# Fe0437/CudaVolumeRenderer

Measured on AMD Instinct MI355X. Metric: Msamples/sec + achieved HBM GB/s, manix.vdb 1024x1024 @ 1/2/4/8 MI355X, higher is better.
Workload: dtype f32

## Files before the change

### cudavolumerenderer_amd/csrc/cvr_wpool.hip

```cpp
#include <hip/hip_runtime.h>

#include "cvr_env.h"
#include "cvr_kernels.h"
#include "cvr_walk.h"

#ifndef CVR_WPOOL_UNROLL
#define CVR_WPOOL_UNROLL 4
#endif
#ifndef CVR_WPOOL_EMASK
#define CVR_WPOOL_EMASK 1
#endif
#ifndef CVR_WPOOL_SPARSE_WPG
#define CVR_WPOOL_SPARSE_WPG 4
#endif
#ifndef CVR_WPOOL_DENSE_WPG
#define CVR_WPOOL_DENSE_WPG 1
#endif
#ifndef CVR_WPOOL_LOOK
#define CVR_WPOOL_LOOK 2
#endif
#ifndef CVR_WPOOL_SPARSE_DEFER
#define CVR_WPOOL_SPARSE_DEFER 1
#endif
#ifndef CVR_WPOOL_TAILSTAMP
#define CVR_WPOOL_TAILSTAMP 0
#endif
constexpr int kLook = CVR_WPOOL_LOOK;
static_assert(CVR_WPOOL_UNROLL >= kLook && CVR_WPOOL_UNROLL % kLook == 0,
              "CVR_WPOOL_UNROLL must be a positive multiple of kLook");
constexpr int kPrioTrack = 1, kPrioEvent = 0;

namespace cvr {

namespace {

__device__ __forceinline__ float opaque_s(float x) {
  asm volatile("" : "+s"(x));
  return x;
}

constexpr int kLdsGranule = 1280;
template <int kWaves, int kExtra = 0, int kWpg = 1>
struct PoolSize {
  static_assert((4 * kWaves) % kWpg == 0, "a CU's waves split into whole workgroups");
  static constexpr int kBudget = 163840 / (4 * kWaves / kWpg) / kLdsGranule * kLdsGranule;
  static constexpr int kParams = (int)((sizeof(LaunchParams) + 15) / 16 * 16);
  static constexpr int value = ((kBudget - kParams - kExtra) / kWpg - 24 - 4 * STAT_COUNT) / 64;
  static_assert(4 * STAT_COUNT + 8 + 12 + 4 <= 4 * STAT_COUNT + 24, "pool header exceeds its LDS reserve");
};
constexpr int kWpgSparse = CVR_WPOOL_SPARSE_WPG, kWpgDense = CVR_WPOOL_DENSE_WPG;
constexpr int wpg_of(int kMedMk, int kWaves) {
  return (kMedMk & 3) != 1  ? ((4 * kWaves) % kWpgDense == 0 ? kWpgDense : 1)
                                            : ((4 * kWaves) % kWpgSparse == 0 ? kWpgSparse : 4);
}

template <int kSlots>
struct WavePool {
  float4 a[kSlots], b[kSlots];
  uint4 c[kSlots];
  uint2 e[kSlots];
  uint32_t meta[kSlots];
  uint8_t ready[kSlots];
  uint8_t lb[kSlots];
  uint8_t lc[kSlots];
  uint8_t ln[kSlots];
  uint32_t cnt[STAT_COUNT];
  unsigned long long dead;
  uint32_t cur[3];
  uint32_t pend;
};
constexpr uint32_t kCurExhausted = 1u << 16;

__device__ __forceinline__ uint32_t lane_rank(unsigned long long mask) {
  return __builtin_amdgcn_mbcnt_hi((uint32_t)(mask >> 32), __builtin_amdgcn_mbcnt_lo((uint32_t)mask, 0u));
}

__device__ __forceinline__ uint32_t normal_code(V3 n) {
  return n.x > 0.f ? 1u : n.x < 0.f ? 2u : n.y > 0.f ? 3u : n.y < 0.f ? 4u : n.z > 0.f ? 5u : n.z < 0.f ? 6u : 0u;
}
__device__ __forceinline__ V3 normal_of(uint32_t c) {
  const float s = (c & 1u) ? 1.0f : -1.0f;
  return c == 0u ? mk3(0, 0, 0) : c <= 2u ? mk3(s, 0, 0) : c <= 4u ? mk3(0, s, 0) : mk3(0, 0, s);
}

template <class Pool>
__device__ __forceinline__ void store_full(Pool& S, float4* __restrict__ gT, uint32_t s,
                                           const PathState& ps, const Isect& is, uint32_t nseg,
                                           uint32_t wword) {
  S.a[s] = make_float4(ps.o.x, ps.o.y, ps.o.z, 0.0f);
  S.b[s] = make_float4(ps.d.x, ps.d.y, ps.d.z, is.dist);
  S.c[s] = make_uint4(ps.rng.v0, ps.rng.v1, ps.rng.v2, ps.rng.v3);
  S.e[s] = make_uint2(ps.rng.v4, ps.rng.d);
  S.meta[s] = normal_code(is.normal) | (is.inside ? 8u : 0u) | (nseg << 4);
  gstore4(gT + s, make_float4(ps.T.x, ps.T.y, ps.T.z, __uint_as_float(wword)));
}
template <class Pool>
__device__ __forceinline__ void load_full(const Pool& S, const float4* __restrict__ gT, uint32_t s,
                                          PathState& ps, Isect& is, uint32_t& nseg, float& t) {
  const float4 f = gload4(gT + s);
  const float4 a = S.a[s], b = S.b[s];
  const uint4 c = S.c[s];
  const uint2 e = S.e[s];
  const uint32_t meta = S.meta[s];
  ps.o = mk3(a.x, a.y, a.z);
  t = a.w;
  ps.d = mk3(b.x, b.y, b.z);
  is.dist = b.w;
  ps.T = mk3(f.x, f.y, f.z);
  ps.rng = Rng{c.x, c.y, c.z, c.w, e.x, e.y};
  ps.image_id = __float_as_uint(f.w);
  is.normal = normal_of(meta & 7u);
  is.inside = (meta & 8u) != 0u;
  nseg = meta >> 4;
}
template <class Pool>
__device__ __forceinline__ void store_track(Pool& S, uint32_t s, float t, const Rng& rng) {
  S.a[s].w = t;
  S.c[s] = make_uint4(rng.v0, rng.v1, rng.v2, rng.v3);
  S.e[s] = make_uint2(rng.v4, rng.d);
}
template <class Pool>
__device__ __forceinline__ void load_track(const Pool& S, uint32_t s, V3& o, V3& d, Rng& rng, float& t,
                                           float& max_t) {
  const float4 a = S.a[s], b = S.b[s];
  const uint4 c = S.c[s];
  const uint2 e = S.e[s];
  o = mk3(a.x, a.y, a.z);
  t = a.w;
  d = mk3(b.x, b.y, b.z);
  max_t = b.w;
  rng = Rng{c.x, c.y, c.z, c.w, e.x, e.y};
}

typedef __attribute__((address_space(3))) const LaunchParams LdsParams;
__device__ __forceinline__ const LaunchParams& fresh(const LaunchParams& L) {
  LdsParams* p = (LdsParams*)&L;
  asm volatile("" : "+v"(p));
  return *(const LaunchParams*)p;
}

enum : uint32_t { K_BOUNDARY = 0, K_COLLIDE = 1, K_NEW = 2, K_NONE = 3 };

template <bool kCombine, class Pool>
__device__ __forceinline__ void splat_wave(Pool& S, const LaunchParams& L, const PathState& ps, bool esc,
                                           uint32_t s, uint32_t lane) {
#if defined(CVR_DIAG_NO_SPLAT)
  (void)S; (void)L; (void)ps; (void)esc; (void)s; (void)lane;
  return;
#endif
  unsigned long long rest = __ballot(esc);
  if (rest == 0ull) return;
  if (!kCombine || !(fresh(L).wflags & kSplatCombine)) {
    if (esc) splat(L, ps);
    return;
  }
  uint32_t leader = lane;
  bool multi = false;
  while (rest != 0ull) {
    const uint32_t l0 = (uint32_t)__builtin_ctzll(rest);
    const uint32_t id0 = __builtin_amdgcn_readlane(ps.image_id, l0);
    const unsigned long long g = __ballot(esc && ps.image_id == id0);
    if (esc && ps.image_id == id0) leader = l0;
    multi |= (g & (g - 1ull)) != 0ull;
    rest &= ~g;
  }
  if (!multi) {
    if (esc) splat(L, ps);
    return;
  }
  const uint32_t sl = (uint32_t)__shfl((int)s, (int)leader);
  float* acc = reinterpret_cast<float*>(&S.a[sl]);
  const bool lead = esc && leader == lane;
  if (lead) {
    acc[0] = ps.T.x;
    acc[1] = ps.T.y;
    acc[2] = ps.T.z;
  }
  asm volatile("s_waitcnt lgkmcnt(0)" ::: "memory");
  if (esc && !lead) {
    __hip_atomic_fetch_add(acc + 0, ps.T.x, __ATOMIC_RELAXED, __HIP_MEMORY_SCOPE_WORKGROUP);
    __hip_atomic_fetch_add(acc + 1, ps.T.y, __ATOMIC_RELAXED, __HIP_MEMORY_SCOPE_WORKGROUP);
    __hip_atomic_fetch_add(acc + 2, ps.T.z, __ATOMIC_RELAXED, __HIP_MEMORY_SCOPE_WORKGROUP);
  }
  asm volatile("s_waitcnt lgkmcnt(0)" ::: "memory");
  if (lead) {
    PathState q{};
    q.image_id = ps.image_id;
    q.T = mk3(acc[0], acc[1], acc[2]);
    splat(L, q);
  }
}

template <int kSlots, int kWpg>
__device__ __forceinline__ uint32_t* rec_pids(const LaunchParams& L, uint32_t gw) {
  return reinterpret_cast<uint32_t*>(L.rec) - (size_t)gridDim.x * kWpg * kSlots + (size_t)gw * kSlots;
}
template <int kSlots, int kWpg>
__device__ __forceinline__ void record_end(const LaunchParams& L, uint32_t gw, uint32_t s, const PathState& ps,
                                           uint32_t flags, uint32_t nseg) {
  const uint32_t pid = rec_pids<kSlots, kWpg>(L, gw)[s];
  PathRecord r = {};
  r.image_id = ps.image_id;
  r.flags = flags;
  r.T[0] = ps.T.x;
  r.T[1] = ps.T.y;
  r.T[2] = ps.T.z;
  r.n_segments = nseg;
  static_cast<PathRecord*>(L.rec)[pid - L.path_first] = r;
}



constexpr unsigned kWaitVm0 = 0x0F70;
constexpr uint32_t kPendAgg = 0x80000000u;

template <class Pool>
__device__ __forceinline__ uint32_t count_ended(const Pool& S, const LaunchParams& L, uint32_t pend,
                                                uint32_t lane) {
#if defined(CVR_DIAG_NO_COUNT)
  (void)S; (void)L; (void)pend; (void)lane;
  return 0u;
#endif
  const uint32_t base = pend & 0xFFu, n = pend >> 8;
#if !defined(CVR_DIAG_NO_COUNT_WAIT)
  __builtin_amdgcn_s_waitcnt(kWaitVm0);
#endif
  uint32_t blk = 0;
  if (lane < n) blk = tile_block_of(fresh(L), S.meta[S.ln[base + lane]]);
  const uint32_t b0 = __builtin_amdgcn_readfirstlane(blk);
  const unsigned long long same = __ballot(lane < n && blk == b0);
  const bool rest = lane < n && blk != b0;
  const unsigned long long rm = __ballot(rest);
  if (rm != 0ull) {
    const uint32_t first = (uint32_t)__builtin_ctzll(rm);
    const uint32_t b1 = __builtin_amdgcn_readlane(blk, first);
    const unsigned long long s1 = __ballot(rest && blk == b1);
    if (lane == first || (rest && blk != b1))
      __hip_atomic_fetch_add(gmem(fresh(L).frame_done + kDoneStride * blk), lane == first ? (unsigned int)__popcll(s1) : 1u,
                             __ATOMIC_RELAXED, __HIP_MEMORY_SCOPE_AGENT);
  }
  return kPendAgg | b0 << 7 | (uint32_t)__popcll(same);
}
__device__ __forceinline__ void add_counted(const LaunchParams& L, uint32_t agg) {
#if defined(CVR_DIAG_NO_COUNT)
  (void)L; (void)agg;
  return;
#endif
  __hip_atomic_fetch_add(gmem(fresh(L).frame_done + kDoneStride * ((agg & ~kPendAgg) >> 7)), agg & 0x7Fu,
                         __ATOMIC_RELAXED, __HIP_MEMORY_SCOPE_AGENT);
}

__device__ __forceinline__ void store_blocks(const LaunchParams& L, const FrameFlush& F, const uint32_t (&b)[8], uint32_t nb,
                                             uint32_t lane) {
  float v[8][3];
  size_t pix[8];
#pragma unroll
  for (uint32_t k = 0; k < 8u; ++k) {
    if (k < nb) {
      const uint32_t by = fastdiv(b[k], L.div_blocks_x), bx = b[k] - by * L.blocks_x;
      const uint32_t px = bx * 8u + (lane & 7u), py = by * 8u + (lane >> 3);
      pix[k] = (size_t)py * L.tile_w + px;
      gptr_t<float> src = gmem(reinterpret_cast<float*>(L.out + pix[k]));
#pragma unroll
      for (int c = 0; c < 3; ++c) v[k][c] = __hip_atomic_fetch_add(src + c, 0.0f, __ATOMIC_RELAXED, __HIP_MEMORY_SCOPE_AGENT);
    }
  }
#pragma unroll
  for (uint32_t k = 0; k < 8u; ++k) {
    if (k < nb) {
      const float x = v[k][0], y = v[k][1], z = v[k][2];
      const float w = (x != 0.0f || y != 0.0f || z != 0.0f) ? 1.0f : 0.0f;
      float4* dst = F.host + pix[k];
      __builtin_nontemporal_store(x / F.scale, &dst->x);
      __builtin_nontemporal_store(y / F.scale, &dst->y);
      __builtin_nontemporal_store(z / F.scale, &dst->z);
      __builtin_nontemporal_store(w / F.scale, &dst->w);
    }
  }
}

constexpr unsigned long long kFlushPatience = 100000000ull;
constexpr unsigned int kFlushed = 0x80000000u;
__device__ void frame_flusher(const LaunchParams& L, uint32_t f, uint32_t lane) {
  const FrameFlush F = *frame_header(L.frame_done);
  if (F.give_up) {
    if (lane == 0) __hip_atomic_store(F.status + kFrameFlushers, 1u, __ATOMIC_RELAXED, __HIP_MEMORY_SCOPE_SYSTEM);
    return;
  }
  const uint32_t quota = 64u * L.samples, qi = lane & 7u, off = lane >> 3, q = f + kFrameFlushers * qi;
  uint32_t cur = 0, end = 0, stored = 0;
  if (q < L.n_queues) {
    cur = queue_blocks_begin(L, q);
    end = queue_blocks_begin(L, q + 1u);
  }
  unsigned long long last = __builtin_amdgcn_s_memrealtime();
  for (;;) {
    if (__ballot(cur < end) == 0ull) break;
    const bool mine = cur + off < end;
    uint32_t tb = 0, v = 0;
    if (mine) {
      tb = launch_block_tile(L, cur + off);
      v = __hip_atomic_fetch_add(gmem(L.frame_done + kDoneStride * tb), 0u, __ATOMIC_RELAXED, __HIP_MEMORY_SCOPE_AGENT);
    }
    const bool ready = mine && v < kFlushed && v >= quota;
    unsigned long long rm = __ballot(ready);
    const unsigned long long settled = __ballot(mine && v >= quota);
    const unsigned long long now = __builtin_amdgcn_s_memrealtime();
    const bool any_ready = rm != 0ull;
    while (rm != 0ull) {
      uint32_t bsel[8], nb = 0;
#pragma unroll
      for (uint32_t k = 0; k < 8u; ++k) {
        if (rm != 0ull) {
          bsel[k] = __builtin_amdgcn_readlane(tb, (uint32_t)__builtin_ctzll(rm));
          rm &= rm - 1ull;
          ++nb;
        }
      }
      store_blocks(L, F, bsel, nb, lane);
      stored += nb;
    }
    if (ready) __hip_atomic_fetch_or(gmem(L.frame_done + kDoneStride * tb), kFlushed, __ATOMIC_RELAXED, __HIP_MEMORY_SCOPE_AGENT);
    uint32_t lead = 0;
#pragma unroll
    for (uint32_t o = 0; o < 8u; ++o)
      if (lead == o && ((settled >> (qi + 8u * o)) & 1ull)) ++lead;
    cur += lead;
    if (any_ready) {
      last = now;
    } else if (__ballot(lead != 0u) == 0ull) {
      if (now - last > kFlushPatience) {
        if (lane == 0) __hip_atomic_store(F.status + kFrameFlushers, 1u, __ATOMIC_RELAXED, __HIP_MEMORY_SCOPE_SYSTEM);
        break;
      }
      __builtin_amdgcn_s_sleep(32);
    }
  }
  if (lane == 0) __hip_atomic_store(F.status + f, stored, __ATOMIC_RELAXED, __HIP_MEMORY_SCOPE_SYSTEM);
}


}

#if CVR_WPOOL_TAILSTAMP
constexpr uint32_t kTailWaves = 16384;
__device__ unsigned long long g_tail[8 * kTailWaves];
#endif
static_assert(sizeof(LaunchParams) == 256 && sizeof(MediumParams) == 256,
              "the moments buffer is addressed from LaunchParams::out: the parameter structs keep their size");
__device__ __forceinline__ void splat_moments(const LaunchParams& L, const PathState& ps) {
  gptr_t<float> px = gmem(reinterpret_cast<float*>(L.out + L.tile_px + ps.image_id));
  const float xx = ps.T.x * ps.T.x, yy = ps.T.y * ps.T.y, zz = ps.T.z * ps.T.z;
  if (xx != 0.0f) __hip_atomic_fetch_add(px + 0, xx, __ATOMIC_RELAXED, __HIP_MEMORY_SCOPE_AGENT);
  if (yy != 0.0f) __hip_atomic_fetch_add(px + 1, yy, __ATOMIC_RELAXED, __HIP_MEMORY_SCOPE_AGENT);
  if (zz != 0.0f) __hip_atomic_fetch_add(px + 2, zz, __ATOMIC_RELAXED, __HIP_MEMORY_SCOPE_AGENT);
  __hip_atomic_fetch_add(px + 3, 1.0f, __ATOMIC_RELAXED, __HIP_MEMORY_SCOPE_AGENT);
}
__device__ __forceinline__ void env_shade(const LaunchParams& L, PathState& ps) {
  typedef __attribute__((address_space(4))) const uint32_t* CWords;
  const uint64_t a = reinterpret_cast<uint64_t>(fresh(L).rec);
  const uint32_t lo = (uint32_t)__builtin_amdgcn_readfirstlane((uint32_t)a);
  const uint32_t hi = (uint32_t)__builtin_amdgcn_readfirstlane((uint32_t)(a >> 32));
  const uint64_t ua = (uint64_t)lo | (uint64_t)hi << 32;
  CWords hw = reinterpret_cast<CWords>(ua);
  EnvParams E;
  E.texels = reinterpret_cast<const float4*>((uint64_t)hw[0] | (uint64_t)hw[1] << 32);
  E.w = hw[2];
  E.h = hw[3];
#pragma unroll
  for (int i = 0; i < 9; ++i) E.R[i] = __uint_as_float(hw[4 + i]);
  float rgb[3];
  env_lookup(E, ps.d.x, ps.d.y, ps.d.z, rgb);
  ps.T = mk3(ps.T.x * rgb[0], ps.T.y * rgb[1], ps.T.z * rgb[2]);
}
template <bool kScatterEps, int kWaves, int kMedMk, bool kRecord, bool kFlush>
__global__ __launch_bounds__(64 * wpg_of(kMedMk, kWaves), kWaves) void k_wpool(MediumParams mk, LaunchParams Lk) {
  constexpr bool kMK = (kMedMk & kMedMK) != 0;
  constexpr bool kCountWords = (kMedMk & kMedCount) != 0;
  constexpr bool kMoments = (kMedMk & kMedMoments) != 0;
  constexpr bool kEnv = (kMedMk & kMedEnv) != 0;
  constexpr int kMed = kMedMk & 3;
  static_assert(!kEnv || (kWaves == kWpoolWaves && !kMK && !kRecord && !kFlush && !kCountWords),
                "environment: the default budget, no naiveMK walk, records, in-launch output or word counts");
  static_assert(!kMoments || (!kMK && !kRecord && !kFlush && !kCountWords && !(kMedMk & kMedHalf)),
                "moments: no naiveMK walk, records, in-launch output, word counts or pinned half format");
  static_assert(!kMK || (kScatterEps && !kRecord && !kFlush), "naiveMK: scatter -eps, no records / in-launch output");
  constexpr bool kSparse = kMed == kMedSparse;
  constexpr bool kLookDefer = kSparse && CVR_WPOOL_SPARSE_DEFER;
  constexpr int kEm = kSparse && CVR_WPOOL_EMASK ? kEmaskWords : 0;
  constexpr int kWpg = wpg_of(kMedMk, kWaves);
  constexpr int kSlots = PoolSize<kWaves, 4 * kEm, kWpg>::value;
  if constexpr (kFlush && kWpg == 1) {
    if (Lk.frame_done != nullptr && blockIdx.x < kFrameFlushers) {
      frame_flusher(Lk, blockIdx.x, threadIdx.x);
      return;
    }
  }
  const uint32_t wv = kWpg > 1 ? __builtin_amdgcn_readfirstlane(threadIdx.x >> 6) : 0u;
  const uint32_t gw = blockIdx.x * (uint32_t)kWpg + wv;
  MediumParams m = mk;
  if constexpr (!kSparse) {
    m.leaves = nullptr;
    m.leaf_density = nullptr;
    m.leaf_albedo = nullptr;
    m.sbounds = nullptr;
    if constexpr (kMed == kMedDenseFull || kMed == kMedDenseFullUniform) {
      __builtin_assume(m.cells != nullptr);
      __builtin_assume(m.bounds != nullptr);
      m.albedo_uniform = kMed == kMedDenseFullUniform ? 1u : 0u;
      m.format = (kMedMk & kMedHalf) ? 1u : 0u;
    }
  } else {
    m.density = nullptr;
    m.albedo = nullptr;
    m.bounds = nullptr;
    __builtin_assume(m.leaves != nullptr);
    __builtin_assume(m.sbounds != nullptr);
    m.albedo_uniform = 0u;
    m.format = (kMedMk & kMedHalf) ? 1u : 0u;
  }
  static_assert(!(kMedMk & kMedHalf) || kMed != kMedDense, "the generic dense instance reads the format at run time");
#if CVR_WPOOL_TAILSTAMP
  const unsigned long long ts_start = __builtin_amdgcn_s_memrealtime();
  unsigned long long ts_ex = 0, ts_ev = 0, ts_a = 0;
  uint32_t ts_live = 0, ts_batches = 0, ts_trk = 0, ts_steps0 = 0, ts_seg0 = 0;
#endif
  static_assert(kWpg * sizeof(WavePool<kSlots>) + 4 * kEm + sizeof(LaunchParams) <=
                    (size_t)PoolSize<kWaves, 0, kWpg>::kBudget,
                "wave pools exceed the LDS budget of kWaves waves per SIMD");
  static_assert(kSlots <= 256, "the pool's rings and stacks hold slot indices as uint8_t");
  __shared__ WavePool<kSlots> Sw[kWpg];
  WavePool<kSlots>& S = Sw[wv];
  __shared__ uint32_t EM[kEm ? kEm : 1];
  __shared__ LaunchParams L;
  const uint32_t lane = kWpg > 1 ? threadIdx.x & 63u : threadIdx.x;
  if (threadIdx.x == 0) L = Lk;
  if constexpr (kEm != 0) {
    for (uint32_t i = threadIdx.x; i < (uint32_t)kEm; i += 64u * kWpg) EM[i] = m.emask ? m.emask[i] : ~0u;
  }
  __syncthreads();
  if constexpr (kFlush && kWpg > 1) {
    if (Lk.frame_done != nullptr && gw < kFrameFlushers) {
      frame_flusher(Lk, gw, lane);
      return;
    }
  }
  uint32_t c_steps = 0, c_fetch = 0;
  uint32_t c_words = 0;
  if (lane < (uint32_t)STAT_COUNT) S.cnt[lane] = 0u;
  if (lane == 0) {
    S.dead = 0ull;
    S.pend = 0u;
  }
  uint32_t n_over = 0;
  if (lane == 0) {
    S.cur[0] = S.cur[1] = 0u;
    S.cur[2] = (((__builtin_amdgcn_s_getreg((3 << 11) | (0 << 6) | 20) & 7u) % (L.n_queues / L.sub)) * L.sub +
                ((blockIdx.x >> 3) * (uint32_t)kWpg + wv) % L.sub)
               << 8;
  }
  const uint32_t batch = L.batch;
  uint32_t ready_head = 0, n_ready = 0, n_lb = 0, n_lc = 0;
  uint32_t n_ln = kSlots;
  for (uint32_t i = lane; i < (uint32_t)kSlots; i += 64u) S.ln[i] = (uint8_t)i;

  for (;;) {
    __builtin_amdgcn_s_setprio(kPrioTrack);
    int slot = -1;
    int fst = 0;
    V3 o = mk3(0, 0, 0), d = mk3(0, 0, 0);
    Rng rng{0, 0, 0, 0, 0, 0};
    float t = 0.0f, max_t = 0.0f;
    const float4* pcp = nullptr;
    float pxt = 0.0f;
    for (;;) {
      const unsigned long long trk = (__ballot(slot >= 0) & __ballot(fst == 0));
      const uint32_t n_trk = (uint32_t)__popcll(trk);
      if (64u - n_trk >= batch || n_trk == 0u) {
        if (fst == 2 && !(t < max_t)) fst = 3;
        if (fst != 0) store_track(S, (uint32_t)slot, t, rng);
        const unsigned long long mc = __ballot(fst == 2), mb = __ballot(fst & 1);
        if (fst == 2) S.lc[n_lc + lane_rank(mc)] = (uint8_t)slot;
        if (fst & 1) S.lb[n_lb + lane_rank(mb)] = (uint8_t)slot;
        n_lc += (uint32_t)__popcll(mc);
        n_lb += (uint32_t)__popcll(mb);
        n_over += (uint32_t)__popcll(__ballot(fst == 1));
        if (fst != 0) {
          slot = -1;
          fst = 0;
        }
        const unsigned long long idle = __ballot(slot < 0);
        const uint32_t k = min((uint32_t)__popcll(idle), n_ready), rank = lane_rank(idle);
        if (slot < 0 && rank < k) {
          const uint32_t r = ready_head + rank;
          const uint32_t s = S.ready[r >= (uint32_t)kSlots ? r - kSlots : r];
          slot = (int)s;
          load_track(S, s, o, d, rng, t, max_t);
        }
        ready_head += k;
        if (ready_head >= (uint32_t)kSlots) ready_head -= kSlots;
        n_ready -= k;
      }
      const uint32_t n_act = (uint32_t)__popcll((__ballot(slot >= 0) & __ballot(fst == 0)));
      const uint32_t n_fin = (uint32_t)__popcll(__ballot(fst != 0));
      if (n_lb + n_lc + n_ln + n_fin >= 64u || (n_act == 0u && n_ready == 0u)) {
        if (fst == 2 && !(t < max_t)) fst = 3;
        if (slot >= 0) store_track(S, (uint32_t)slot, t, rng);
        const unsigned long long mr = (__ballot(slot >= 0) & __ballot(fst == 0));
        const unsigned long long mc = __ballot(fst == 2), mb = __ballot(fst & 1);
        if (slot >= 0 && fst == 0) S.ready[(ready_head + n_ready + lane_rank(mr)) % kSlots] = (uint8_t)slot;
        if (fst == 2) S.lc[n_lc + lane_rank(mc)] = (uint8_t)slot;
        if (fst & 1) S.lb[n_lb + lane_rank(mb)] = (uint8_t)slot;
        n_over += (uint32_t)__popcll(__ballot(fst == 1));
        n_ready += (uint32_t)__popcll(mr);
        n_lc += (uint32_t)__popcll(mc);
        n_lb += (uint32_t)__popcll(mb);
        break;
      }
#pragma unroll
      for (int u = 0; u < CVR_WPOOL_UNROLL / kLook; ++u) {
        if (slot >= 0 && fst == 0) {
          float tk[kLook], xtk[kLook];
          uint32_t sva[kLook], svb[kLook];
          WoodcockPoint Pk[kLook];
          float tt = t;
#pragma unroll
          for (int k = 0; k < kLook; ++k) {
            const float xi = rng_float(rng);
            xtk[k] = rng_float(rng);
            sva[k] = rng.v0;
            svb[k] = rng.v1;
            tt = woodcock_advance(m, xi, tt);
            tk[k] = tt;
          }
#pragma unroll
          for (int k = 0; k < kLook; ++k) {
            if constexpr (kEm != 0)
              Pk[k] = woodcock_point_em<kEm>(m, o, d, tk[k], EM, kCountWords ? &c_words : nullptr);
            else
              Pk[k] = woodcock_point(m, o, d, tk[k]);
          }
          int end = kLook;
#pragma unroll
          for (int k = 0; k < kLook; ++k) {
            if (end == kLook) {
              if (!(tk[k] <= max_t)) {
                fst = 1;
                end = k;
              } else if (!(Pk[k].qb < xtk[k])) {
                if constexpr (kLookDefer) {
                  fst = 4;
                  end = k;
                  pcp = Pk[k].cp;
                  pxt = xtk[k];
                } else {
                  ++c_fetch;
                  const float rho = m.scale * woodcock_density(m, Pk[k]);
                  if (!(rho * m.inv_sigma < xtk[k])) {
                    fst = 2;
                    end = k;
                  }
                }
              }
            }
          }
          c_steps += end == kLook ? kLook : end + 1;
          t = tk[kLook - 1];
#pragma unroll
          for (int k = 0; k < kLook - 1; ++k)
            if (end == k) t = tk[k];
          if (end < kLook - 1) {
            uint32_t w[2 * kLook + 5];
#pragma unroll
            for (int k = 0; k < kLook - 1; ++k) {
              w[2 * k + 2] = sva[k];
              w[2 * k + 3] = svb[k];
            }
            w[2 * kLook] = rng.v0;
            w[2 * kLook + 1] = rng.v1;
            w[2 * kLook + 2] = rng.v2;
            w[2 * kLook + 3] = rng.v3;
            w[2 * kLook + 4] = rng.v4;
#pragma unroll
            for (int j = 1; j < kLook; ++j) {
              if (end + 1 == j) {
                rng.v0 = w[2 * j];
                rng.v1 = w[2 * j + 1];
                rng.v2 = w[2 * j + 2];
                rng.v3 = w[2 * j + 3];
                rng.v4 = w[2 * j + 4];
              }
            }
            rng.d -= (uint32_t)(2 * (kLook - 1 - end)) * 362437u;
          }
        }
      }
      if constexpr (kLookDefer) {
        if (fst == 4) {
          ++c_fetch;
          WoodcockPoint P;
          woodcock_coords(m, o, d, t, P);
          P.cp = pcp;
          const float rho = m.scale * woodcock_density(m, P);
          fst = !(rho * m.inv_sigma < pxt) ? 2 : 0;
        }
      }
    }
    if (n_lb + n_lc == 0u && n_ready == 0u && (n_ln == 0u || (S.cur[2] & kCurExhausted))) break;

    __builtin_amdgcn_s_setprio(kPrioEvent);
#if CVR_WPOOL_TAILSTAMP
    if (ts_ex != 0) ts_a = __builtin_amdgcn_s_memrealtime();
#endif
    if constexpr (kFlush) {
      const uint32_t pend = S.pend;
      if (pend != 0u) {
        const uint32_t agg = count_ended(S, L, pend, lane);
        if (lane == 0) S.pend = agg;
      }
    }
    MediumParams me = m;
    me.g = opaque_s(m.g);
    me.ax = opaque_s(m.ax);
    me.ay = opaque_s(m.ay);
    me.eta = opaque_s(m.eta);
    me.inv_eta = opaque_s(m.inv_eta);
    me.bmin = mk3(opaque_s(m.bmin.x), opaque_s(m.bmin.y), opaque_s(m.bmin.z));
    me.bmax = mk3(opaque_s(m.bmax.x), opaque_s(m.bmax.y), opaque_s(m.bmax.z));
    me.albedo_bg = mk3(opaque_s(m.albedo_bg.x), opaque_s(m.albedo_bg.y), opaque_s(m.albedo_bg.z));
    if constexpr (kMed == kMedDense)
      me.albedo_uniform = __float_as_uint(opaque_s(__uint_as_float(m.albedo_uniform)));
    {
#ifndef CVR_WPOOL_KIND_MIN
#define CVR_WPOOL_KIND_MIN 48
#endif
#ifndef CVR_WPOOL_KIND_MIN_C
#define CVR_WPOOL_KIND_MIN_C 24
#endif
      uint32_t tb, tc, tn;
      if (n_lb >= (uint32_t)CVR_WPOOL_KIND_MIN) {
        tb = min(n_lb, 64u);
        tc = 0;
        tn = min(n_ln, 64u - tb);
      } else if (n_lc >= (uint32_t)CVR_WPOOL_KIND_MIN_C) {
        tb = 0;
        tc = min(n_lc, 64u);
        tn = n_ln < 64u ? 0u : min(n_ln, 64u - tc);
      } else {
        tb = min(n_lb, 64u);
        tc = min(n_lc, 64u - tb);
        tn = min(n_ln, 64u - tb - tc);
      }
      uint32_t kind = K_NONE, s = 0;
      if (lane < tb) {
        kind = K_BOUNDARY;
        s = S.lb[n_lb - 1u - lane];
      } else if (lane < tb + tc) {
        kind = K_COLLIDE;
        s = S.lc[n_lc - 1u - (lane - tb)];
      } else if (lane < tb + tc + tn) {
        kind = K_NEW;
        s = S.ln[n_ln - 1u - (lane - tb - tc)];
      }
      n_lb -= tb;
      n_lc -= tc;
      n_ln -= tn;
      PathState ps{};
      Isect is{};
      uint32_t nseg = 0;
      uint32_t mk_pid = 0;
      float t_hit = 0.0f;
      bool to_ready = false, to_lb = false, to_ln = false;
      bool alive = false;
      bool truncated = false, escaped = false, seg_first = false, seg_next = false;
      const unsigned long long want = __ballot(kind == K_NEW);
      if (want != 0ull) {
        const uint32_t rank = lane_rank(want);
        bool got = false;
        uint32_t given = 0;
        uint32_t cnext = __builtin_amdgcn_readfirstlane(S.cur[0]), cend = __builtin_amdgcn_readfirstlane(S.cur[1]);
        uint32_t cqh = __builtin_amdgcn_readfirstlane(S.cur[2]);
        while (given < (uint32_t)__popcll(want) && !(cqh & kCurExhausted)) {
          if (cnext == cend) {
            uint32_t b = 0xFFFFFFFFu, qsel = 0;
            if (lane == 0) {
              unsigned long long dead = S.dead;
              for (uint32_t k = 0; k < L.n_queues; ++k) {
                const uint32_t q = ((cqh >> 8) + k) % L.n_queues;
                if ((dead >> q) & 1ull) continue;
                const uint32_t g = atomicAdd(L.queue + 16 * q, L.chunk);
                if (g < queue_units(L, q)) {
                  b = g;
                  qsel = q;
                  break;
                }
                dead |= 1ull << q;
              }
              S.dead = dead;
            }
            b = __shfl(b, 0);
            qsel = __shfl(qsel, 0);
            if (b == 0xFFFFFFFFu) {
              cqh |= kCurExhausted;
              break;
            }
            cqh = qsel | qsel << 8;
            cnext = b;
            cend = min(b + L.chunk, queue_units(L, qsel));
          }
          const uint32_t take = min((uint32_t)__popcll(want) - given, cend - cnext);
          if (kind == K_NEW && rank >= given && rank < given + take) {
            const uint32_t pid = unit_to_path(L, cqh & 0xFFu, cnext + (rank - given));
            if constexpr (kMK) {
              mk_pid = pid;
            } else {
              path_begin(L, pid, ps);
            }
            if (kRecord) rec_pids<kSlots, kWpg>(L, gw)[s] = pid;
            is.normal = mk3(0, 0, 0);
            nseg = 0;
            got = true;
          }
          cnext += take;
          given += take;
        }
        if (lane == 0) {
          S.cur[0] = cnext;
          S.cur[1] = cend;
          S.cur[2] = cqh;
        }
        const uint32_t n_got = (uint32_t)__popcll(__ballot(got));
        if (lane == 0) S.cnt[STAT_PATHS] += n_got;
        if constexpr (kMK) {
          if (got) {
            const uint32_t it = fastdiv(mk_pid, L.div_tile_px);
            nseg = 1;
            seg_first = true;
            const uint32_t r0 = mk_init(me, L, it, mk_pid - it * L.tile_px, ps);
            if (r0 == MK_MISSED) {
              escaped = true;
              to_ln = true;
            } else if (r0 == MK_DROPPED) {
              to_ln = true;
            } else {
              alive = true;
            }
          }
        } else if (got) {
          if (L.max_segments && nseg >= L.max_segments) {
            truncated = true;
            to_ln = true;
            if (kFlush) S.meta[s] = ps.image_id;
            if (kRecord) record_end<kSlots, kWpg>(L, gw, s, ps, 2u, nseg);
          } else {
            ++nseg;
            seg_first = true;
            if (!aabb_intersect(me, ps.o, ps.d, is)) {
              escaped = true;
              to_ln = true;
              if (kFlush) S.meta[s] = ps.image_id;
              if (kRecord) record_end<kSlots, kWpg>(L, gw, s, ps, 1u, nseg);
            } else if (is.inside) {
              store_full(S, L.pool_T + (size_t)(kWpg > 1 ? gw : blockIdx.x) * kSlots, s, ps, is, nseg, ps.image_id);
              to_ready = true;
            } else {
              kind = K_BOUNDARY;
            }
          }
        }
      }
      float4* __restrict__ gT = L.pool_T + (size_t)(kWpg > 1 ? gw : blockIdx.x) * kSlots;
      if (lane < tb + tc) {
        load_full(S, gT, s, ps, is, nseg, t_hit);
        if constexpr (kMK) {
          mk_pid = ps.image_id;
          ps.image_id = mk_pid - fastdiv(mk_pid, L.div_tile_px) * L.tile_px;
        }
      }
      if (lane < tb && !(t_hit <= is.dist)) rng_undo(ps.rng);
      if (kind == K_BOUNDARY) {
        boundary_event(me, ps, is);
        alive = roulette(ps);
      }
      if (kind == K_COLLIDE) {
        scatter_event<kScatterEps>(me, ps, t_hit);
        alive = roulette(ps);
      }
      const uint32_t n_alb = (uint32_t)__popcll(__ballot(kind == K_COLLIDE));
      if ((kind == K_BOUNDARY || kind == K_COLLIDE) && !alive) {
        to_ln = true;
        if (kFlush) S.meta[s] = ps.image_id;
        if (kRecord) record_end<kSlots, kWpg>(L, gw, s, ps, 0u, nseg);
      }
      if (alive) {
        if (L.max_segments && nseg >= L.max_segments) {
          truncated = true;
          to_ln = true;
          if (kFlush) S.meta[s] = ps.image_id;
          if (kRecord) record_end<kSlots, kWpg>(L, gw, s, ps, 2u, nseg);
        } else {
          ++nseg;
          seg_next = true;
          if constexpr (kMK) {
            const uint32_t it = fastdiv(mk_pid, L.div_tile_px);
            rng_seeded(ps.rng, it, ps.image_id, nseg - 2u);
            (void)rng_float(ps.rng);
            (void)rng_float(ps.rng);
            (void)rng_float(ps.rng);
            is.dist = 0.0f;
            is.normal = mk3(0, 0, 0);
            is.inside = false;
          }
          if (!aabb_intersect(me, ps.o, ps.d, is)) {
            escaped = true;
            to_ln = true;
            if (kFlush) S.meta[s] = ps.image_id;
            if (kRecord) record_end<kSlots, kWpg>(L, gw, s, ps, 1u, nseg);
          } else {
            store_full(S, gT, s, ps, is, nseg, kMK ? mk_pid : ps.image_id);
            to_ready = is.inside;
            to_lb = !is.inside;
          }
        }
      }
      if constexpr (kEnv) {
        if (escaped) env_shade(L, ps);
      }
      splat_wave<!kFlush && !kMoments>(S, L, ps, escaped, s, lane);
      if constexpr (kMoments) {
        if (escaped) splat_moments(L, ps);
      }
      {
        const uint32_t n_seg = (uint32_t)(__popcll(__ballot(seg_first)) + __popcll(__ballot(seg_next)));
        const uint32_t n_esc = (uint32_t)__popcll(__ballot(escaped)), n_tr = (uint32_t)__popcll(__ballot(truncated));
        if (lane == 0) {
          S.cnt[STAT_SEGMENTS] += n_seg;
          S.cnt[STAT_ALBEDO] += n_alb;
          S.cnt[STAT_ESCAPED] += n_esc;
          S.cnt[STAT_TRUNCATED] += n_tr;
        }
      }
      const unsigned long long mr = __ballot(to_ready), mb = __ballot(to_lb), mn = __ballot(to_ln);
      if (to_ready) S.ready[(ready_head + n_ready + lane_rank(mr)) % kSlots] = (uint8_t)s;
      if (to_lb) S.lb[n_lb + lane_rank(mb)] = (uint8_t)s;
      if (to_ln) S.ln[n_ln + lane_rank(mn)] = (uint8_t)s;
      if constexpr (kFlush) {
        if (lane == 0) {
          const uint32_t agg = S.pend;
          if (agg != 0u) add_counted(L, agg);
          if (agg != 0u || mn != 0ull)
            S.pend = mn != 0ull ? n_ln | (uint32_t)__popcll(mn) << 8 : 0u;
        }
      }
      n_ready += (uint32_t)__popcll(mr);
      n_lb += (uint32_t)__popcll(mb);
      n_ln += (uint32_t)__popcll(mn);
    }
    if (S.cur[2] & kCurExhausted) {
      const uint32_t n_live = n_ready + n_lb + n_lc;
#if CVR_WPOOL_TAILSTAMP
      if (ts_ex == 0) {
        ts_ex = __builtin_amdgcn_s_memrealtime();
        ts_live = n_live;
        ts_steps0 = c_steps;
        ts_seg0 = S.cnt[STAT_SEGMENTS];
      } else {
        ts_ev += __builtin_amdgcn_s_memrealtime() - ts_a;
      }
      ++ts_batches;
#endif
      {
        const uint32_t d = fresh(L).wflags & kDrainMask;
        n_ln = d ? 64u - min(64u, (n_live * d + d) / (d + 1u)) : 0u;
      }
    }
  }

#if CVR_WPOOL_TAILSTAMP
  {
    const unsigned long long ts_end = __builtin_amdgcn_s_memrealtime();
    uint32_t dsteps = c_steps - ts_steps0;
#pragma unroll
    for (int off = 32; off > 0; off >>= 1) dsteps += __shfl_xor(dsteps, off);
    if (lane == 0 && gw < kTailWaves) {
      const uint32_t xcc = __builtin_amdgcn_s_getreg((3 << 11) | (0 << 6) | 20) & 7u;
      unsigned long long* g = g_tail + 8 * gw;
      g[0] = ts_start;
      g[1] = ts_ex;
      g[2] = ts_end;
      g[3] = (unsigned long long)ts_live | (unsigned long long)ts_batches << 16 | (unsigned long long)xcc << 40;
      g[4] = ts_ev;
      g[5] = dsteps;
      g[6] = S.cnt[STAT_SEGMENTS] - ts_seg0;
      g[7] = ts_trk;
    }
  }
#endif
  if constexpr (kFlush) {
    const uint32_t pend = S.pend;
    if (pend != 0u) {
      const uint32_t agg = count_ended(S, L, pend, lane);
      if (lane == 0) add_counted(L, agg);
    }
  }
  {
    unsigned long long steps = c_steps, fetch = c_fetch;
#pragma unroll
    for (int off = 32; off > 0; off >>= 1) {
      steps += __shfl_xor(steps, off);
      fetch += __shfl_xor(fetch, off);
    }
    const unsigned long long w[STAT_COUNT] = {S.cnt[STAT_PATHS], S.cnt[STAT_SEGMENTS], steps, steps - n_over,
                                              S.cnt[STAT_ALBEDO], S.cnt[STAT_ESCAPED], S.cnt[STAT_TRUNCATED], fetch};
    if (lane < (uint32_t)STAT_COUNT && w[lane])
      __hip_atomic_fetch_add(gmem(L.stats + lane), w[lane], __ATOMIC_RELAXED, __HIP_MEMORY_SCOPE_AGENT);
    if constexpr (kCountWords) {
      unsigned long long words = c_words;
#pragma unroll
      for (int off = 32; off > 0; off >>= 1) words += __shfl_xor(words, off);
      if (lane == 0) __hip_atomic_fetch_add(gmem(L.stats + kStatWordsSlot), words, __ATOMIC_RELAXED, __HIP_MEMORY_SCOPE_AGENT);
    }
  }
}

struct WpoolRow { WpoolInstance id; void (*fn)(MediumParams, LaunchParams); uint32_t wpg, slots; };
constexpr int em_bytes_of(int med) { return (med & 3) == kMedSparse && CVR_WPOOL_EMASK ? 4 * kEmaskWords : 0; }
#define CVR_WP_ROW(E, W, M, R, F) \
  {{E, W, (M), R, F}, &k_wpool<E, W, (M), R, F>, wpg_of((M), W), PoolSize<W, em_bytes_of(M), wpg_of((M), W)>::value}
#define CVR_WP_ROWS(W, M, R, F) CVR_WP_ROW(false, W, M, R, F), CVR_WP_ROW(true, W, M, R, F)
#define CVR_WP_ROWS5(M) CVR_WP_ROWS(5, M, false, false), CVR_WP_ROWS(5, M, false, true)
#define CVR_WP_ROWMK(M) CVR_WP_ROW(true, 5, (M) | kMedMK, false, false)
constexpr WpoolRow kWpoolTable[] = {
    CVR_WP_ROWS5(kMedDense), CVR_WP_ROWS5(kMedSparse), CVR_WP_ROWS5(kMedDenseFull), CVR_WP_ROWS5(kMedDenseFullUniform),
    CVR_WP_ROWS5(kMedSparse | kMedHalf), CVR_WP_ROWS5(kMedDenseFull | kMedHalf),
    CVR_WP_ROWS5(kMedDenseFullUniform | kMedHalf),
    CVR_WP_ROWS(3, kMedDense, false, false), CVR_WP_ROWS(4, kMedDense, false, false),
    CVR_WP_ROWS(6, kMedDense, false, false), CVR_WP_ROWS(4, kMedSparse, false, false),
    CVR_WP_ROWS(5, kMedDense, true, false), CVR_WP_ROWS(5, kMedSparse, true, false),
    CVR_WP_ROWS(5, kMedSparse | kMedHalf, true, false), CVR_WP_ROWS(4, kMedSparse, true, false),
    CVR_WP_ROWS(5, kMedDense | kMedMoments, false, false), CVR_WP_ROWS(5, kMedSparse | kMedMoments, false, false),
    CVR_WP_ROWS(5, kMedSparse | kMedCount, false, false),
    CVR_WP_ROWS(5, kMedDense | kMedEnv, false, false), CVR_WP_ROWS(5, kMedSparse | kMedEnv, false, false),
    CVR_WP_ROWS(5, kMedSparse | kMedHalf | kMedEnv, false, false),
    CVR_WP_ROWS(5, kMedDense | kMedEnv | kMedMoments, false, false),
    CVR_WP_ROWS(5, kMedSparse | kMedEnv | kMedMoments, false, false),
    CVR_WP_ROWMK(kMedDense), CVR_WP_ROWMK(kMedSparse), CVR_WP_ROWMK(kMedDenseFull), CVR_WP_ROWMK(kMedDenseFullUniform),
    CVR_WP_ROWMK(kMedSparse | kMedHalf), CVR_WP_ROWMK(kMedDenseFull | kMedHalf),
    CVR_WP_ROWMK(kMedDenseFullUniform | kMedHalf),
};
#undef CVR_WP_ROWMK
#undef CVR_WP_ROWS5
#undef CVR_WP_ROWS
#undef CVR_WP_ROW
constexpr int kWpoolRows = (int)(sizeof(kWpoolTable) / sizeof(kWpoolTable[0]));
constexpr const WpoolRow* wpool_row(const WpoolInstance& k) {
  for (const WpoolRow& r : kWpoolTable)
    if (r.id == k) return &r;
  return nullptr;
}
constexpr bool wpool_table_is_the_selection() {
  bool hit[kWpoolRows] = {};
  WpoolInstance k{};
  for (int i = 0; i < kWpoolRequestsAll; ++i)
    if (wpool_select(wpool_request_at(i), &k)) {
      const WpoolRow* r = wpool_row(k);
      if (!r) return false;
      hit[r - kWpoolTable] = true;
    }
  for (bool h : hit)
    if (!h) return false;
  return true;
}
static_assert(kWpoolRows == 67 && wpool_table_is_the_selection(), "the instance table and wpool_select disagree");

hipError_t launch_wpool(const MediumParams& m, const LaunchParams& L, const WpoolRequest& q, uint32_t grid,
                        hipStream_t s) {
  if (L.path_count == 0) return hipSuccess;
  WpoolInstance k{};
  if (!wpool_select(q, &k)) return hipErrorInvalidValue;
  const WpoolRow& row = *wpool_row(k);
  if (grid % row.wpg) return hipErrorInvalidValue;
  void* args[] = {const_cast<MediumParams*>(&m), const_cast<LaunchParams*>(&L)};
  return hipLaunchKernel(reinterpret_cast<const void*>(row.fn), dim3(grid / row.wpg), dim3(64 * row.wpg), args, 0, s);
}

#if CVR_WPOOL_TAILSTAMP
extern "C" int cvr_debug_tailstamps(unsigned long long* host, size_t n_waves) {
  if (n_waves > kTailWaves) n_waves = kTailWaves;
  return hipMemcpyFromSymbol(host, HIP_SYMBOL(g_tail), n_waves * 64, 0, hipMemcpyDeviceToHost) == hipSuccess ? 0 : -2;
}
extern "C" int cvr_debug_tailstamps_clear() {
  void* p = nullptr;
  if (hipGetSymbolAddress(&p, HIP_SYMBOL(g_tail)) != hipSuccess) return -2;
  return hipMemset(p, 0, sizeof(unsigned long long) * 8 * kTailWaves) == hipSuccess ? 0 : -2;
}
#endif

uint32_t wpool_wpg(const WpoolInstance& k) { return wpool_row(k)->wpg; }
uint32_t wpool_slots(const WpoolInstance& k) { return wpool_row(k)->slots; }
hipError_t wpool_occupancy(const WpoolInstance& k, int* waves_per_cu) {
  const WpoolRow& row = *wpool_row(k);
  const void* fn = reinterpret_cast<const void*>(row.fn);
  const hipError_t e = hipOccupancyMaxActiveBlocksPerMultiprocessor(waves_per_cu, fn, 64 * row.wpg, 0);
  *waves_per_cu *= (int)row.wpg;
  return e;
}

}
```

Before: 5386.

## Add burst path-regeneration phase that filters AABB misses before occupying pool slots

```diff
diff --git a/cudavolumerenderer_amd/csrc/cvr_regen_plan.h b/cudavolumerenderer_amd/csrc/cvr_regen_plan.h
--- /dev/null
+++ b/cudavolumerenderer_amd/csrc/cvr_regen_plan.h
@@ -0,0 +1,63 @@
+#pragma once
+#include <cstdint>
+
+namespace cvr {
+
+constexpr uint32_t kRegenLanes = 64;
+
+struct RegenBurst {
+  uint32_t accepted;
+  uint32_t committed;
+};
+
+constexpr uint32_t regen_width(uint32_t free, uint32_t remaining, uint32_t over) {
+  const uint32_t want = free > kRegenLanes / over ? kRegenLanes : free * over;
+  const uint32_t w = want < kRegenLanes ? want : kRegenLanes;
+  return w < remaining ? w : remaining;
+}
+
+constexpr uint32_t regen_popcount(uint64_t m) { return (uint32_t)__builtin_popcountll(m); }
+
+constexpr uint32_t regen_nth_set(uint64_t m, uint32_t n) {
+  uint32_t pos = 0;
+  for (uint32_t w = 32; w != 0; w >>= 1) {
+    const uint32_t c = regen_popcount((m >> pos) & ((1ull << w) - 1ull));
+    if (n >= c) {
+      n -= c;
+      pos += w;
+    }
+  }
+  return pos;
+}
+
+constexpr RegenBurst regen_plan(uint64_t hits, uint32_t width, uint32_t free) {
+  const uint64_t h = width >= kRegenLanes ? hits : hits & ((1ull << width) - 1ull);
+  const uint32_t n = regen_popcount(h);
+  if (n <= free) return RegenBurst{n, width};
+  return RegenBurst{free, regen_nth_set(h, free)};
+}
+
+constexpr bool regen_plan_holds(uint64_t hits, uint32_t width, uint32_t free) {
+  const RegenBurst b = regen_plan(hits, width, free);
+  if (b.accepted > free || b.committed > width) return false;
+  if (width != 0 && free != 0 && b.committed == 0) return false;
+  uint32_t in = 0;
+  for (uint32_t l = 0; l < b.committed; ++l) in += (uint32_t)((hits >> l) & 1ull);
+  if (in != b.accepted) return false;
+  if (b.committed < width && !(((hits >> b.committed) & 1ull) && b.accepted == free)) return false;
+  return true;
+}
+constexpr bool regen_plan_sweep() {
+  for (uint32_t width = 0; width <= 6; ++width)
+    for (uint32_t free = 0; free <= 7; ++free)
+      for (uint64_t m = 0; m < (1ull << width); ++m)
+        if (!regen_plan_holds(m, width, free)) return false;
+  return regen_plan_holds(~0ull, 64, 64) && regen_plan_holds(~0ull, 64, 1) && regen_plan_holds(1ull << 63, 64, 0) &&
+         regen_nth_set(1ull << 63, 0) == 63 && regen_nth_set(~0ull, 37) == 37;
+}
+static_assert(regen_plan_sweep(), "regen_plan: a burst's accepted hits and committed units disagree");
+static_assert(regen_width(1, 256, 2) == 2 && regen_width(40, 256, 2) == 64 && regen_width(115, 3, 2) == 3 &&
+                  regen_width(0, 9, 2) == 0 && regen_width(5, 0, 2) == 0 && regen_width(3, 256, 64) == 64,
+              "regen_width");
+
+}
diff --git a/cudavolumerenderer_amd/csrc/cvr_wpool.hip b/cudavolumerenderer_amd/csrc/cvr_wpool.hip
--- a/cudavolumerenderer_amd/csrc/cvr_wpool.hip
+++ b/cudavolumerenderer_amd/csrc/cvr_wpool.hip
@@ -2,6 +2,7 @@
 
 #include "cvr_env.h"
 #include "cvr_kernels.h"
+#include "cvr_regen_plan.h"
 #include "cvr_walk.h"
 
 #ifndef CVR_WPOOL_UNROLL
@@ -24,6 +25,18 @@
 #endif
 #ifndef CVR_WPOOL_TAILSTAMP
 #define CVR_WPOOL_TAILSTAMP 0
+#endif
+#ifndef CVR_WPOOL_REGEN_PHASE
+#define CVR_WPOOL_REGEN_PHASE 1
+#endif
+#ifndef CVR_WPOOL_REGEN_OVER
+#define CVR_WPOOL_REGEN_OVER 2
+#endif
+#ifndef CVR_WPOOL_REGEN_MIN
+#define CVR_WPOOL_REGEN_MIN 32
+#endif
+#ifndef CVR_WPOOL_REGENSTAT
+#define CVR_WPOOL_REGENSTAT 0
 #endif
 constexpr int kLook = CVR_WPOOL_LOOK;
 static_assert(CVR_WPOOL_UNROLL >= kLook && CVR_WPOOL_UNROLL % kLook == 0,
@@ -209,7 +222,71 @@
   static_cast<PathRecord*>(L.rec)[pid - L.path_first] = r;
 }
 
-
+__device__ __forceinline__ void record_miss(const LaunchParams& L, uint32_t pid, const PathState& ps) {
+  PathRecord r = {};
+  r.image_id = ps.image_id;
+  r.flags = 1u;
+  r.T[0] = ps.T.x;
+  r.T[1] = ps.T.y;
+  r.T[2] = ps.T.z;
+  r.n_segments = 1u;
+  static_cast<PathRecord*>(L.rec)[pid - L.path_first] = r;
+}
+
+template <class Pool>
+__device__ __forceinline__ void splat_misses(Pool& S, const LaunchParams& L, const PathState& ps, bool esc,
+                                             uint32_t n_free, uint32_t lane) {
+#if defined(CVR_DIAG_NO_SPLAT)
+  (void)S; (void)L; (void)ps; (void)esc; (void)n_free; (void)lane;
+  return;
+#endif
+  unsigned long long rest = __ballot(esc);
+  if (rest == 0ull) return;
+  if (!(fresh(L).wflags & kSplatCombine)) {
+    if (esc) splat(L, ps);
+    return;
+  }
+  uint32_t leader = lane;
+  bool multi = false;
+  while (rest != 0ull) {
+    const uint32_t l0 = (uint32_t)__builtin_ctzll(rest);
+    const uint32_t id0 = __builtin_amdgcn_readlane(ps.image_id, l0);
+    const unsigned long long g = __ballot(esc && ps.image_id == id0);
+    if (esc && ps.image_id == id0) leader = l0;
+    multi |= (g & (g - 1ull)) != 0ull;
+    rest &= ~g;
+  }
+  if (!multi) {
+    if (esc) splat(L, ps);
+    return;
+  }
+  const bool lead = esc && leader == lane;
+  const uint32_t lr = lane_rank(__ballot(lead));
+  uint32_t sl = 0xFFFFFFFFu;
+  if (lead && lr < n_free) sl = S.ln[n_free - 1u - lr];
+  sl = (uint32_t)__shfl((int)sl, (int)leader);
+  const bool comb = esc && sl != 0xFFFFFFFFu;
+  if (esc && !comb) splat(L, ps);
+  float* acc = reinterpret_cast<float*>(&S.a[comb ? sl : 0u]);
+  if (comb && lead) {
+    acc[0] = ps.T.x;
+    acc[1] = ps.T.y;
+    acc[2] = ps.T.z;
+  }
+  asm volatile("s_waitcnt lgkmcnt(0)" ::: "memory");
+  if (comb && !lead) {
+    __hip_atomic_fetch_add(acc + 0, ps.T.x, __ATOMIC_RELAXED, __HIP_MEMORY_SCOPE_WORKGROUP);
+    __hip_atomic_fetch_add(acc + 1, ps.T.y, __ATOMIC_RELAXED, __HIP_MEMORY_SCOPE_WORKGROUP);
+    __hip_atomic_fetch_add(acc + 2, ps.T.z, __ATOMIC_RELAXED, __HIP_MEMORY_SCOPE_WORKGROUP);
+  }
+  asm volatile("s_waitcnt lgkmcnt(0)" ::: "memory");
+  if (comb && lead) {
+    PathState q{};
+    q.image_id = ps.image_id;
+    q.T = mk3(acc[0], acc[1], acc[2]);
+    splat(L, q);
+  }
+}
 
 constexpr unsigned kWaitVm0 = 0x0F70;
 constexpr uint32_t kPendAgg = 0x80000000u;
@@ -346,6 +423,10 @@
 constexpr uint32_t kTailWaves = 16384;
 __device__ unsigned long long g_tail[8 * kTailWaves];
 #endif
+#if CVR_WPOOL_REGENSTAT
+constexpr int kRegenStats = 12;
+__device__ unsigned long long g_regen[kRegenStats];
+#endif
 static_assert(sizeof(LaunchParams) == 256 && sizeof(MediumParams) == 256,
               "the moments buffer is addressed from LaunchParams::out: the parameter structs keep their size");
 __device__ __forceinline__ void splat_moments(const LaunchParams& L, const PathState& ps) {
@@ -380,6 +461,7 @@
   constexpr bool kMoments = (kMedMk & kMedMoments) != 0;
   constexpr bool kEnv = (kMedMk & kMedEnv) != 0;
   constexpr int kMed = kMedMk & 3;
+  constexpr bool kBurst = CVR_WPOOL_REGEN_PHASE && !kMK && !kFlush && !kMoments && !kEnv;
   static_assert(!kEnv || (kWaves == kWpoolWaves && !kMK && !kRecord && !kFlush && !kCountWords),
                 "environment: the default budget, no naiveMK walk, records, in-launch output or word counts");
   static_assert(!kMoments || (!kMK && !kRecord && !kFlush && !kCountWords && !(kMedMk & kMedHalf)),
@@ -452,6 +534,9 @@
     S.dead = 0ull;
     S.pend = 0u;
   }
+#if CVR_WPOOL_REGENSTAT
+  uint32_t rs[kRegenStats] = {};
+#endif
   uint32_t n_over = 0;
   if (lane == 0) {
     S.cur[0] = S.cur[1] = 0u;
@@ -462,6 +547,7 @@
   const uint32_t batch = L.batch;
   uint32_t ready_head = 0, n_ready = 0, n_lb = 0, n_lc = 0;
   uint32_t n_ln = kSlots;
+  uint32_t n_lt = kSlots;
   for (uint32_t i = lane; i < (uint32_t)kSlots; i += 64u) S.ln[i] = (uint8_t)i;
 
   for (;;) {
@@ -503,7 +589,7 @@
       }
       const uint32_t n_act = (uint32_t)__popcll((__ballot(slot >= 0) & __ballot(fst == 0)));
       const uint32_t n_fin = (uint32_t)__popcll(__ballot(fst != 0));
-      if (n_lb + n_lc + n_ln + n_fin >= 64u || (n_act == 0u && n_ready == 0u)) {
+      if (n_lb + n_lc + (kBurst ? n_lt : n_ln) + n_fin >= 64u || (n_act == 0u && n_ready == 0u)) {
         if (fst == 2 && !(t < max_t)) fst = 3;
         if (slot >= 0) store_track(S, (uint32_t)slot, t, rng);
         const unsigned long long mr = (__ballot(slot >= 0) & __ballot(fst == 0));
@@ -630,6 +716,102 @@
     me.albedo_bg = mk3(opaque_s(m.albedo_bg.x), opaque_s(m.albedo_bg.y), opaque_s(m.albedo_bg.z));
     if constexpr (kMed == kMedDense)
       me.albedo_uniform = __float_as_uint(opaque_s(__uint_as_float(m.albedo_uniform)));
+#if CVR_WPOOL_REGENSTAT
+    if (!(S.cur[2] & kCurExhausted)) {
+      rs[6] += n_ln;
+      ++rs[7];
+    }
+#endif
+    if constexpr (kBurst) {
+      uint32_t cqh = __builtin_amdgcn_readfirstlane(S.cur[2]);
+      if (cqh & kCurExhausted) {
+        n_ln = 0u;
+      } else if (n_ln >= (uint32_t)CVR_WPOOL_REGEN_MIN || (n_ln != 0u && n_ready == 0u)) {
+        uint32_t cnext = __builtin_amdgcn_readfirstlane(S.cur[0]), cend = __builtin_amdgcn_readfirstlane(S.cur[1]);
+        float4* __restrict__ gTn = L.pool_T + (size_t)(kWpg > 1 ? gw : blockIdx.x) * kSlots;
+#if CVR_WPOOL_REGENSTAT
+        ++rs[10];
+#endif
+#pragma nounroll
+        for (uint32_t pass = 0; pass < 2u; ++pass) {
+          if (cnext == cend) {
+            uint32_t b = 0xFFFFFFFFu, qsel = 0;
+            if (lane == 0) {
+              unsigned long long dead = S.dead;
+              for (uint32_t k = 0; k < L.n_queues; ++k) {
+                const uint32_t q = ((cqh >> 8) + k) % L.n_queues;
+                if ((dead >> q) & 1ull) continue;
+                const uint32_t g = atomicAdd(L.queue + 16 * q, L.chunk);
+                if (g < queue_units(L, q)) {
+                  b = g;
+                  qsel = q;
+                  break;
+                }
+                dead |= 1ull << q;
+              }
+              S.dead = dead;
+            }
+            b = __shfl(b, 0);
+            qsel = __shfl(qsel, 0);
+            if (b == 0xFFFFFFFFu) {
+              cqh |= kCurExhausted;
+              break;
+            }
+            cqh = qsel | qsel << 8;
+            cnext = b;
+            cend = min(b + L.chunk, queue_units(L, qsel));
+          }
+          const uint32_t W = regen_width(n_ln, cend - cnext, (uint32_t)CVR_WPOOL_REGEN_OVER);
+          const bool cut = W < regen_width(n_ln, kRegenLanes, (uint32_t)CVR_WPOOL_REGEN_OVER);
+          PathState ps{};
+          Isect is{};
+          uint32_t pid = 0;
+          bool hit = false;
+          if (lane < W) {
+            pid = unit_to_path(L, cqh & 0xFFu, cnext + lane);
+            path_begin(L, pid, ps);
+            hit = aabb_intersect(me, ps.o, ps.d, is);
+          }
+          const unsigned long long hits = __ballot(hit);
+          const RegenBurst B = regen_plan(hits, W, n_ln);
+          const bool acc = hit && lane < B.committed, miss = !hit && lane < B.committed;
+          if (kRecord && miss) record_miss(L, pid, ps);
+          splat_misses(S, L, ps, miss, n_ln, lane);
+          asm volatile("" ::: "memory");
+          uint32_t s = 0;
+          if (acc) {
+            s = S.ln[n_ln - 1u - lane_rank(hits)];
+            store_full(S, gTn, s, ps, is, 1u, ps.image_id);
+            if (kRecord) rec_pids<kSlots, kWpg>(L, gw)[s] = pid;
+          }
+          const unsigned long long mi = __ballot(acc && is.inside), mo = __ballot(acc && !is.inside);
+          if (acc && is.inside) S.ready[(ready_head + n_ready + lane_rank(mi)) % kSlots] = (uint8_t)s;
+          if (acc && !is.inside) S.lb[n_lb + lane_rank(mo)] = (uint8_t)s;
+          n_ready += (uint32_t)__popcll(mi);
+          n_lb += (uint32_t)__popcll(mo);
+          n_ln -= B.accepted;
+          cnext += B.committed;
+          if (lane == 0) {
+            S.cnt[STAT_PATHS] += B.committed;
+            S.cnt[STAT_SEGMENTS] += B.committed;
+            S.cnt[STAT_ESCAPED] += B.committed - B.accepted;
+          }
+#if CVR_WPOOL_REGENSTAT
+          ++rs[1];
+          rs[4] += B.accepted;
+          rs[5] += B.committed - B.accepted;
+          rs[8] += W;
+          rs[9] += W - B.committed;
+#endif
+          if (!cut || n_ln == 0u) break;
+        }
+        if (lane == 0) {
+          S.cur[0] = cnext;
+          S.cur[1] = cend;
+          S.cur[2] = cqh;
+        }
+      }
+    }
     {
 #ifndef CVR_WPOOL_KIND_MIN
 #define CVR_WPOOL_KIND_MIN 48
@@ -637,20 +819,31 @@
 #ifndef CVR_WPOOL_KIND_MIN_C
 #define CVR_WPOOL_KIND_MIN_C 24
 #endif
+#ifndef CVR_WPOOL_KIND_MIN_C_PHASE
+#define CVR_WPOOL_KIND_MIN_C_PHASE 32
+#endif
+      constexpr uint32_t kKindMinC = kBurst ? CVR_WPOOL_KIND_MIN_C_PHASE : CVR_WPOOL_KIND_MIN_C;
+      const uint32_t n_new = kBurst ? 0u : n_ln;
       uint32_t tb, tc, tn;
       if (n_lb >= (uint32_t)CVR_WPOOL_KIND_MIN) {
         tb = min(n_lb, 64u);
         tc = 0;
-        tn = min(n_ln, 64u - tb);
-      } else if (n_lc >= (uint32_t)CVR_WPOOL_KIND_MIN_C) {
+        tn = min(n_new, 64u - tb);
+      } else if (n_lc >= kKindMinC) {
         tb = 0;
         tc = min(n_lc, 64u);
-        tn = n_ln < 64u ? 0u : min(n_ln, 64u - tc);
+        tn = n_new < 64u ? 0u : min(n_new, 64u - tc);
       } else {
         tb = min(n_lb, 64u);
         tc = min(n_lc, 64u - tb);
-        tn = min(n_ln, 64u - tb - tc);
-      }
+        tn = min(n_new, 64u - tb - tc);
+      }
+#if CVR_WPOOL_REGENSTAT
+      ++rs[0];
+      rs[2] += tb;
+      rs[3] += tc;
+      if (!kBurst) rs[4] += tn;
+#endif
       uint32_t kind = K_NONE, s = 0;
       if (lane < tb) {
         kind = K_BOUNDARY;
@@ -673,8 +866,11 @@
       bool to_ready = false, to_lb = false, to_ln = false;
       bool alive = false;
       bool truncated = false, escaped = false, seg_first = false, seg_next = false;
-      const unsigned long long want = __ballot(kind == K_NEW);
+      const unsigned long long want = kBurst ? 0ull : __ballot(kind == K_NEW);
       if (want != 0ull) {
+#if CVR_WPOOL_REGENSTAT
+        ++rs[1];
+#endif
         const uint32_t rank = lane_rank(want);
         bool got = false;
         uint32_t given = 0;
@@ -832,6 +1028,9 @@
       }
       {
         const uint32_t n_seg = (uint32_t)(__popcll(__ballot(seg_first)) + __popcll(__ballot(seg_next)));
+#if CVR_WPOOL_REGENSTAT
+        rs[5] += (uint32_t)__popcll(__ballot(seg_first && escaped));
+#endif
         const uint32_t n_esc = (uint32_t)__popcll(__ballot(escaped)), n_tr = (uint32_t)__popcll(__ballot(truncated));
         if (lane == 0) {
           S.cnt[STAT_SEGMENTS] += n_seg;
@@ -873,6 +1072,9 @@
         const uint32_t d = fresh(L).wflags & kDrainMask;
         n_ln = d ? 64u - min(64u, (n_live * d + d) / (d + 1u)) : 0u;
       }
+      if constexpr (kBurst) n_lt = n_ln;
+    } else if constexpr (kBurst) {
+      n_lt = n_ln >= (uint32_t)CVR_WPOOL_REGEN_MIN ? n_ln : 0u;
     }
   }
 
@@ -903,6 +1105,13 @@
       if (lane == 0) add_counted(L, agg);
     }
   }
+#if CVR_WPOOL_REGENSTAT
+  if (lane == 0) {
+#pragma unroll
+    for (int k = 0; k < kRegenStats; ++k)
+      if (rs[k]) __hip_atomic_fetch_add(g_regen + k, (unsigned long long)rs[k], __ATOMIC_RELAXED, __HIP_MEMORY_SCOPE_AGENT);
+  }
+#endif
   {
     unsigned long long steps = c_steps, fetch = c_fetch;
 #pragma unroll
@@ -996,6 +1205,16 @@
 }
 #endif
 
+#if CVR_WPOOL_REGENSTAT
+extern "C" int cvr_debug_regenstats(unsigned long long* host, int clear) {
+  void* p = nullptr;
+  if (hipGetSymbolAddress(&p, HIP_SYMBOL(g_regen)) != hipSuccess) return -2;
+  if (hipMemcpy(host, p, sizeof(unsigned long long) * kRegenStats, hipMemcpyDeviceToHost) != hipSuccess) return -2;
+  if (clear && hipMemset(p, 0, sizeof(unsigned long long) * kRegenStats) != hipSuccess) return -2;
+  return kRegenStats;
+}
+#endif
+
 uint32_t wpool_wpg(const WpoolInstance& k) { return wpool_row(k)->wpg; }
 uint32_t wpool_slots(const WpoolInstance& k) { return wpool_row(k)->slots; }
 hipError_t wpool_occupancy(const WpoolInstance& k, int* waves_per_cu) {
```

Result: faster. 5452, median of 6 (+1.2%).
